# vrenkens/tfkaldi

Hardware: AMD Instinct MI355X
Metric: acoustic frames/sec (train step) (higher is better)
Workload: dtype f32 emulated (3xbf16 planes, 6 products, f32 accumulate)

## Files before the change

### tfkaldi_amd/csrc/engine.hip

```cpp
#include "../../include/tfkaldi_hip.h"
#include "ctc.h"
#include "gemm_bf16.h"
#include "gemm_f32.h"
#include "kernels.h"

#include <hip/hip_runtime.h>
#include <chrono>

#include <math.h>
#include <stdarg.h>
#include <stdlib.h>
#include <stdio.h>
#include <string.h>

#include <algorithm>
#include <string>
#include <vector>

using namespace tfk;

namespace {

thread_local std::string g_err;

// ... 61 lines not shown
  std::vector<hipEvent_t> ev_adam;
  bool opt_overlap = false;
  bool opt_pending = false;
  float* d_snap = nullptr;
  hipEvent_t ev_loss = nullptr;
  unsigned loss_seq = 0;
  bool loss_event = false;
  bool slot_lazy = true;
  hipEvent_t ev_grow = nullptr;
  std::vector<void*> host_garbage;

  float* state = nullptr;
  bool own_state = false;
  size_t P = 0, E = 0, state_floats = 0;
  size_t off_param = 0, off_grad = 0, off_scalars = 0, off_ema = 0, off_m = 0, off_v = 0, off_mov = 0, off_shadow = 0;
  size_t reduce_floats = 0;
  std::vector<LayerLayout> lay;

  int cap = 0;
  float* dX[2] = {nullptr, nullptr};
  int32_t* dY[2] = {nullptr, nullptr};
  std::vector<float*> z, a, v, rowscale, mean, rstd;
  float *logits = nullptr, *post = nullptr, *dA[2] = {nullptr, nullptr}, *row_loss = nullptr, *ws = nullptr;
  float* dRaw[2] = {nullptr, nullptr};
  int32_t* dSeg[2] = {nullptr, nullptr};
  float* hRaw[2] = {nullptr, nullptr};
  int32_t* hSeg[2] = {nullptr, nullptr};
  float* dCmvn[2] = {nullptr, nullptr};
  float* hCmvn[2] = {nullptr, nullptr};
  size_t cmvn_cap = 0;
  int seg_cap = 0;
  std::vector<float*> seg_mean, seg_rstd;
  float* ws_stats = nullptr;
  float* ws_bwd = nullptr;
  float* ws_splitk = nullptr;
  size_t ws_splitk_floats = 0;
  size_t ws_bwd_stride = 0;
  float* prior = nullptr;
  bool have_prior = false;

  float* hX[2] = {nullptr, nullptr};
  int32_t* hY[2] = {nullptr, nullptr};
  float* h_post = nullptr;
  size_t h_post_floats = 0;
  float* h_scalars = nullptr;
  float* h_scalars_dev = nullptr;
  bool apply_open = false, apply_direct = false;
  float cur_lr_t = 0.f;
  bool scalars_fresh = true;
  bool step_open = false;
  bool stash_live = false;
  float* scalar_stash = nullptr;
  bool colsum_done = false;
  bool fuse_hb_enabled = true;
  bool dual_gemm = true;
  bool stack_enabled = true;
  bool fuse_eval = true;
  int post_chunk = 2048;
  std::vector<hipEvent_t> post_ev;

  int32_t *ctc_seg = nullptr, *ctc_lab_off = nullptr, *ctc_lab = nullptr;
  float *ctc_lp = nullptr, *ctc_ab = nullptr, *ctc_bb = nullptr, *ctc_utt_loss = nullptr, *ctc_lse = nullptr;
  double *ctc_off = nullptr, *ctc_offb = nullptr, *ctc_logz = nullptr;
  size_t ctc_cap_bb = 0, ctc_cap_offb = 0, ctc_cap_logz = 0;
  int32_t* h_ctc[2] = {nullptr, nullptr};
  size_t h_ctc_cap[2] = {0, 0};
  hipEvent_t ctc_staged[2] = {nullptr, nullptr};
  int ctc_stage_slot = 0;
  size_t ctc_cap_offrows = 0;
  size_t ctc_cap_seg = 0, ctc_cap_off = 0, ctc_cap_loss = 0, ctc_cap_lab = 0, ctc_cap_lp = 0, ctc_cap_ab = 0,
         ctc_cap_rows = 0;
  int32_t* ctc_dec = nullptr;
  size_t ctc_cap_dec = 0;
  int32_t* h_dec = nullptr;
  size_t h_dec_cap = 0;
  unsigned long long* ctc_trie = nullptr;
  size_t ctc_cap_trie = 0;
  uint32_t* ctc_pre = nullptr;
  size_t ctc_cap_pre = 0;
  float* ctc_lm = nullptr;
  int ctc_lm_order = 0;
  unsigned char* ctc_bp = nullptr;
  size_t ctc_cap_bp = 0;
  unsigned char* ctc_sc = nullptr;
  size_t ctc_cap_sc = 0;
  int32_t* ctc_pair = nullptr;
  size_t ctc_cap_pair = 0;
  int32_t* h_pair = nullptr;
  size_t h_pair_cap = 0;
  hipEvent_t ctc_pair_staged = nullptr;

  bool bf16 = false;
  bool x3 = false;
  size_t tw_elems(size_t rows, int ld) const { return x3 ? x3::elems(rows, ld) : rows * ld; }
  size_t tw_row(size_t r, int ld) const { return x3 ? x3::at(r, 0, ld) : r * ld; }
  ShadowMap wb_map;
  int ldFb = 0, ldHb = 0, ldOb = 0;
  bf16_t* Xb[2] = {nullptr, nullptr};
  std::vector<bf16_t*> ab;
  bf16_t* logb = nullptr;
  bf16_t* dAb[2] = {nullptr, nullptr};
  bf16_t* Wb = nullptr;
  std::vector<size_t> wb_off;
  std::vector<int> wb_ld;
  bool wb_aligned = false;
  bool own_wb = false;
// ... 340 lines not shown
  auto frb = [&](bf16_t*& p) { dev_free(e, p, async); p = nullptr; };
  for (int s = 0; s < 2; ++s) { frb(e->Xb[s]); frb(e->dAb[s]); }
  for (auto& p : e->ab) frb(p);
  frb(e->logb);
  for (auto& p : e->z) fr(p);
  for (auto& p : e->a) fr(p);
  for (auto& p : e->v) fr(p);
  for (auto& p : e->rowscale) fr(p);
  fr(e->logits); fr(e->post); fr(e->row_loss); fr(e->ws); fr(e->ws_bwd); fr(e->ws_stats);
  e->cap = 0;
}

int alloc_zero(float** p, size_t floats) {
  HIPCHK(hipMalloc((void**)p, floats * sizeof(float)));
  HIPCHK(hipMemset(*p, 0, floats * sizeof(float)));
  HIPCHK(hipStreamSynchronize(nullptr));
  return 0;
}
int alloc_zero_b(bf16_t** p, size_t elems) {
  HIPCHK(hipMalloc((void**)p, elems * sizeof(bf16_t)));
  HIPCHK(hipMemset(*p, 0, elems * sizeof(bf16_t)));
  HIPCHK(hipStreamSynchronize(nullptr));
  return 0;
}
int grow_zero(tfk_engine* e, float** p, size_t floats) { return dev_alloc(e, (void**)p, floats * sizeof(float), true); }
int grow_zero_b(tfk_engine* e, bf16_t** p, size_t elems) { return dev_alloc(e, (void**)p, elems * sizeof(bf16_t), true); }

inline size_t seg_ints(int cap) { return (size_t)2 * cap + cap / 64 + 8; }

int reserve(tfk_engine* e, int T) {
  if (T <= e->cap) return 0;
  int cap = e->cap + e->cap / 2;
  if (cap < T) cap = T;
  cap = (int)up(cap, 64);
  for (int s = 0; s < 2; ++s)
    if (e->slot_used[s]) HIPCHK(hipEventSynchronize(e->copy_done[s]));
  free_activations(e, true);
  const int L = e->L;
  for (int s = 0; s < 2; ++s) {
    CHK(grow_zero(e, &e->dX[s], (size_t)cap * e->ldF));
    CHK(dev_alloc(e, (void**)&e->dY[s], (size_t)cap * sizeof(int32_t), false));
    CHK(grow_zero(e, &e->dA[s], (size_t)cap * e->ldH));
    HIPCHK(hipHostMalloc((void**)&e->hX[s], (size_t)cap * e->F * sizeof(float), hipHostMallocDefault));
    memset(e->hX[s], 0, (size_t)cap * e->F * sizeof(float));
    HIPCHK(hipHostMalloc((void**)&e->hY[s], (size_t)cap * sizeof(int32_t), hipHostMallocDefault));
    CHK(grow_zero(e, &e->dRaw[s], (size_t)cap * e->ldF));
    CHK(dev_alloc(e, (void**)&e->dSeg[s], seg_ints(cap) * sizeof(int32_t), false));
    HIPCHK(hipHostMalloc((void**)&e->hRaw[s], (size_t)cap * e->F * sizeof(float), hipHostMallocDefault));
    memset(e->hRaw[s], 0, (size_t)cap * e->F * sizeof(float));
    HIPCHK(hipHostMalloc((void**)&e->hSeg[s], seg_ints(cap) * sizeof(int32_t), hipHostMallocDefault));
    e->slot_used[s] = false;
  }
  e->z.assign(L, nullptr); e->a.assign(L, nullptr); e->v.assign(L, nullptr); e->rowscale.assign(L, nullptr);
  for (int l = 0; l < L; ++l) {
    CHK(grow_zero(e, &e->z[l], (size_t)cap * e->ldH));
    CHK(grow_zero(e, &e->a[l], (size_t)cap * e->ldH));
    if (e->cfg.l2_norm) {
      CHK(grow_zero(e, &e->v[l], (size_t)cap * e->ldH));
      CHK(grow_zero(e, &e->rowscale[l], (size_t)cap));
    }
  }
  if (e->bf16) {
    for (int s = 0; s < 2; ++s) {
      CHK(grow_zero_b(e, &e->Xb[s], e->tw_elems(cap, e->ldFb)));
      CHK(grow_zero_b(e, &e->dAb[s], e->tw_elems(cap, e->ldHb)));
    }
    e->ab.assign(L, nullptr);
    for (int l = 0; l < L; ++l) CHK(grow_zero_b(e, &e->ab[l], e->tw_elems(cap, e->ldHb)));
    CHK(grow_zero_b(e, &e->logb, e->tw_elems(cap, e->ldOb)));
  }
  CHK(grow_zero(e, &e->logits, (size_t)cap * e->ldO));
  CHK(grow_zero(e, &e->post, (size_t)cap * e->ldO));
  CHK(grow_zero(e, &e->row_loss, (size_t)cap));
  const int ldmax = e->ldH > e->ldO ? e->ldH : e->ldO;
  CHK(grow_zero(e, &e->ws, (size_t)3 * kMaxRowSplits * ldmax));
  CHK(grow_zero(e, &e->ws_stats, (size_t)2 * ((cap + 63) / 64) * e->ldH));
  e->ws_bwd_stride = (size_t)3 * kMaxRowSplits * ldmax;
  CHK(grow_zero(e, &e->ws_bwd, e->ws_bwd_stride * (L + 1)));
  HIPCHK(hipEventRecord(e->ev_grow, e->stream));
  HIPCHK(hipStreamWaitEvent(e->copy_stream, e->ev_grow, 0));
  e->cap = cap;
  return 0;
}

constexpr int kMaxStack = 32;
struct Stack {
  int k = 0;
  int r0[kMaxStack], rows[kMaxStack], span[kMaxStack];
  int T_pad = 0, T_valid = 0;
  const int* d_vend = nullptr;
};
int stack_align(const tfk_engine* e) { return (e->bf16 && !e->x3) ? 256 : 128; }

int wait_slot_free(tfk_engine* e, int s);
int stage_input(tfk_engine* e, const float* X, int64_t ldx, const int32_t* y, int T, int flags, const float** Xd,
                int* ldx_out, const int32_t** yd) {
  if (ldx < e->F) return fail(-1, "ldx %lld < input_dim %d", (long long)ldx, e->F);
  if (flags & TFK_DEVICE_PTRS) {
    if ((ldx % 4) == 0 && (e->F % 4) == 0 && (((uintptr_t)X) % 16) == 0) {
      *Xd = X;
      *ldx_out = (int)ldx;
    } else {
      const int s = e->slot;
      HIPCHK(hipMemcpy2DAsync(e->dX[s], (size_t)e->ldF * 4, X, (size_t)ldx * 4, (size_t)e->F * 4, T,
                              hipMemcpyDeviceToDevice, e->stream));
      *Xd = e->dX[s];
// ... 104 lines not shown
                  cmvn ? e->dCmvn[s] : nullptr, e->dX[s], e->ldF, st ? e->dSeg[s] + U + 1 : nullptr);
  }
  if (st) st->d_vend = e->dSeg[s] + 2 * U + 1;
  e->slot_used[s] = true;
  *Xd = e->dX[s];
  *ldx_out = e->ldF;
  *yd = e->dY[s];
  e->slot ^= 1;
  return 0;
}

int twin_input(tfk_engine* e, const float** Xd, int* ld, int T) {
  int s = (*Xd == e->dX[0]) ? 0 : (*Xd == e->dX[1]) ? 1 : -1;
  const float* src = *Xd;
  const int ld_src = *ld;
  if (s < 0) {
    s = e->slot;
    *Xd = e->dX[s];
    *ld = e->ldF;
  }
  to_bf16_rows(e->stream, src, ld_src, e->Xb[s], e->ldFb, T, e->F, e->x3);
  HIPCHK(hipGetLastError());
  return 0;
}

int finish_slot(tfk_engine* e, int flags, int slot_before) {
  if ((flags & TFK_DEVICE_PTRS) || e->slot == slot_before) return 0;
  if ((flags & TFK_LAST_MICROBATCH) && e->slot_lazy) {
    e->slot_step[slot_before] = e->steps_begun + 1;
    return 0;
  }
  e->slot_step[slot_before] = 0;
  HIPCHK(hipEventRecord(e->compute_done[slot_before], e->stream));
  return 0;
}
int wait_slot_free(tfk_engine* e, int s) {
  if (!e->slot_used[s]) return 0;
  if (e->slot_step[s] == 0) {
    HIPCHK(hipStreamWaitEvent(e->copy_stream, e->compute_done[s], 0));
  } else if (e->steps_seen < e->slot_step[s]) {
    HIPCHK(hipStreamSynchronize(e->stream));
  }
  return 0;
}

ActDesc act_desc(const tfk_engine* e, int layer, int train, uint32_t call) {
  ActDesc d;
  d.nonlin = e->cfg.nonlin; d.bn = e->cfg.batch_norm ? 1 : 0; d.l2 = e->cfg.l2_norm ? 1 : 0;
  d.keep = e->dropout ? e->cfg.keep_prob : 1.f;
  d.seed = e->cfg.seed; d.call = call; d.layer = (uint32_t)layer; d.train = train;
  return d;
}

int forward(tfk_engine* e, const float* Xd, int ldx, int T, int train, int nact, int nfw, uint32_t call,
            const Stack* st = nullptr) {
  const float* in = Xd;
  int ld_in = ldx;
  const int H = e->H, ldH = e->ldH;
  if (e->bf16 && e->shadow_dirty) {
    need_params(e, -1);
    CHK(join_optimizer(e));
    CHK(refresh_shadow(e));
  }
  auto twin_a = [&](int l) { Twin t; if (e->bf16) { t.p = e->ab[l]; t.ld = e->ldHb; t.x3 = e->x3; } return t; };
  for (int l = 0; l < nfw; ++l) {
    const LayerLayout& y = e->lay[l];
    need_params(e, l);
    CHK(wait_layer_update(e, l, l == 0));
    if (train && e->cfg.batch_norm && !e->cfg.l2_norm) {
      int cfg;
      const int chunk = gemm_chunk_rows(e, GEMM_NN, T, H, y.d_in, &cfg);
      if (st && stack_align(e) % chunk) return fail(-1, "internal: GEMM tile of %d rows does not divide the stack alignment", chunk);
      CHK(run_gemm(e, GEMM_NN, in, ld_in, e->p_param() + y.w_off, y.ld_out, e->z[l], ldH, T, H, y.d_in,
                   e->p_param() + y.b_off, EPI_BIAS | EPI_COLSTATS, nullptr, e->ws_stats, cfg, nullptr, st ? st->d_vend : nullptr));
      const int nchunk = (T + chunk - 1) / chunk;
      if (st) {
        for (int i = 0; i < st->k; ++i) {
          ProfScope ps(e, KF_ACT_FWD, 0, 8.0 * st->rows[i] * H);
          const ActDesc d = act_desc(e, l, train, call + (uint32_t)i);
          Twin tw = twin_a(l);
          if (e->bf16) tw.p += e->tw_row((size_t)st->r0[i], e->ldHb);
          bn_act_forward(e->stream, d, e->z[l] + (size_t)st->r0[i] * ldH, e->a[l] + (size_t)st->r0[i] * ldH,
                         e->ws_stats + (size_t)(st->r0[i] / chunk) * ldH, chunk, st->rows[i], H, ldH, e->bn_eps, e->bn_decay,
                         e->seg_mean[l] + (size_t)i * ldH, e->seg_rstd[l] + (size_t)i * ldH, e->ema_mean(l), e->ema_var(l),
                         e->p_param() + y.beta_off, tw, st->span[i], nchunk);
        }
      } else {
        ProfScope ps(e, KF_ACT_FWD, 0, 8.0 * T * H);
        const ActDesc d = act_desc(e, l, train, call);
        if (nchunk > kMergeOnceChunks && nchunk <= kMaxRowSplits) {
          bn_stats_from_chunks(e->stream, e->ws_stats, chunk, T, H, ldH, e->bn_eps, e->bn_decay, e->mean[l], e->rstd[l],
                               e->ema_mean(l), e->ema_var(l));
          act_forward(e->stream, d, e->z[l], e->a[l], nullptr, nullptr, e->mean[l], e->rstd[l],
                      e->p_param() + y.beta_off, T, H, ldH, twin_a(l));
        } else {
          bn_act_forward(e->stream, d, e->z[l], e->a[l], e->ws_stats, chunk, T, H, ldH, e->bn_eps,
                         e->bn_decay, e->mean[l], e->rstd[l], e->ema_mean(l), e->ema_var(l),
                         e->p_param() + y.beta_off, twin_a(l));
        }
      }
      in = e->a[l];
      ld_in = ldH;
      continue;
    }
    if (!train && !e->cfg.l2_norm && e->fuse_eval) {
      ActEpi ev = {nullptr, nullptr, e->cfg.batch_norm ? e->mov_mean(l) : nullptr,
                   e->cfg.batch_norm ? e->mov_var(l) : nullptr, e->cfg.nonlin};
      ev.beta = e->cfg.batch_norm ? e->p_param() + y.beta_off : nullptr;
      ev.eps = e->bn_eps;
      if (e->bf16) { ev.twin = e->ab[l]; ev.ld_twin = e->ldHb; }
      CHK(run_gemm(e, GEMM_NN, in, ld_in, e->p_param() + y.w_off, y.ld_out, e->a[l], ldH, T, H, y.d_in,
                   e->p_param() + y.b_off, EPI_BIAS | EPI_EVAL_ACT, nullptr, nullptr, -1, &ev));
      in = e->a[l];
      ld_in = ldH;
      continue;
    }
    CHK(run_gemm(e, GEMM_NN, in, ld_in, e->p_param() + y.w_off, y.ld_out, e->z[l], ldH, T, H, y.d_in,
                 e->p_param() + y.b_off, EPI_BIAS));
    if (e->cfg.batch_norm) {
      ProfScope ps(e, KF_BN_STATS, 0, 8.0 * T * H);
      if (train)
        bn_stats_train(e->stream, e->z[l], T, H, ldH, e->bn_eps, e->bn_decay, e->mean[l], e->rstd[l], e->ema_mean(l),
                       e->ema_var(l), e->ws);
      else
        bn_stats_eval(e->stream, e->mov_mean(l), e->mov_var(l), H, e->bn_eps, e->mean[l], e->rstd[l]);
    }
    {
      ProfScope ps(e, KF_ACT_FWD, 0, 8.0 * T * H);
      const ActDesc d = act_desc(e, l, train, call);
      act_forward(e->stream, d, e->z[l], e->a[l], e->cfg.l2_norm ? e->v[l] : nullptr,
                  e->cfg.l2_norm ? e->rowscale[l] : nullptr, e->mean[l], e->rstd[l],
                  e->cfg.batch_norm ? e->p_param() + y.beta_off : nullptr, T, H, ldH, twin_a(l));
    }
    in = e->a[l];
    ld_in = ldH;
  }
  const LayerLayout& o = e->lay[e->L];
  need_params(e, e->L);
  CHK(wait_layer_update(e, e->L, nfw == 0));
  CHK(run_gemm(e, GEMM_NN, e->a[nact - 1], ldH, e->p_param() + o.w_off, o.ld_out, e->logits, e->ldO, T, e->O, H,
               e->p_param() + o.b_off, EPI_BIAS));
  HIPCHK(hipGetLastError());
  return 0;
}

int backward(tfk_engine* e, const float* Xd, int ldx, int T, int nact, uint32_t call, bool fire, const Stack* st = nullptr) {
  const int L = e->L, H = e->H, ldH = e->ldH;
  const LayerLayout& o = e->lay[L];
  float* G = e->p_grad();
  const int acc = e->grads_fresh ? 0 : 1;
  const int epi_w = acc ? EPI_ACCUM : 0;
  if (!acc)
    for (int l = nact; l < L; ++l) {
      const LayerLayout& q = e->lay[l];
      HIPCHK(hipMemsetAsync(G + q.w_off, 0, q.w_sz * sizeof(float), e->stream));
      HIPCHK(hipMemsetAsync(G + q.b_off, 0, q.b_sz * sizeof(float), e->stream));
      if (q.beta_sz) HIPCHK(hipMemsetAsync(G + q.beta_off, 0, q.beta_sz * sizeof(float), e->stream));
    }
  FinalBatch fin;
  fin.n = 0;
  fin.accumulate = acc;
  const int rs = row_splits(T);
  auto ws_of = [&](int l) { return e->ws_bwd + (size_t)l * e->ws_bwd_stride; };
  {
    if (!e->colsum_done) {
      ProfScope ps(e, KF_COLSUM, 0, 4.0 * T * e->O);
      colsum_partial(e->stream, e->logits, T, e->ldO, ws_of(L));
    }
    e->colsum_done = false;
    fin.it[fin.n++] = {ws_of(L), G + o.b_off, 0, rs, e->O, e->ldO};
  }
  int pp = 0;
  int cfg_h, cfg_o;
  const int rows_h = gemm_chunk_rows(e, GEMM_NT, T, H, H, &cfg_h), rows_o = gemm_chunk_rows(e, GEMM_NT, T, H, e->O, &cfg_o);
  const bool drop = e->cfg.keep_prob < 1.f;
  const bool fuse_hb = e->cfg.batch_norm && !e->cfg.l2_norm && (!drop || e->cfg.nonlin == TFK_NONLIN_RELU) &&
                       e->fuse_hb_enabled && (T + rows_h - 1) / rows_h <= kMaxRowSplits &&
                       (T + rows_o - 1) / rows_o <= kMaxRowSplits;
  const std::vector<float*>& mean = st ? e->seg_mean : e->mean;
  const std::vector<float*>& rstd = st ? e->seg_rstd : e->rstd;
  auto act_of = [&](int l) {
    ActEpi act = {e->a[l], e->z[l], mean[l], rstd[l], e->cfg.nonlin};
    act.scale = drop ? 1.f / e->cfg.keep_prob : 1.f;
    act.beta = e->cfg.batch_norm ? e->p_param() + e->lay[l].beta_off : nullptr;
    return act;
  };
  auto dact_gemm = [&](const float* dz, int ld_dz, const float* W, int ldw, float* out, int K, int target, int cfg) {
    if (!fuse_hb) return run_gemm(e, GEMM_NT, dz, ld_dz, W, ldw, out, ldH, T, H, K, nullptr, 0);
    const ActEpi act = act_of(target);
    return run_gemm(e, GEMM_NT, dz, ld_dz, W, ldw, out, ldH, T, H, K, nullptr, EPI_DACT, nullptr, ws_of(target), cfg, &act);
  };
  int bm_in = rows_o;
  {
    const ActEpi act = act_of(nact - 1);
    const int rc = run_gemm_dual(e, e->logits, e->ldO, e->p_param() + o.w_off, o.ld_out, e->dA[pp], ldH, T, H, e->O,
                                 fuse_hb ? &act : nullptr, fuse_hb ? ws_of(nact - 1) : nullptr, e->a[nact - 1], ldH,
                                 G + o.w_off, o.ld_out, H, e->O, epi_w, &bm_in);
    if (rc < 0) return rc;
    if (rc > 0) {
      CHK(run_gemm(e, GEMM_TN, e->a[nact - 1], ldH, e->logits, e->ldO, G + o.w_off, o.ld_out, H, e->O, T, nullptr, epi_w));
      CHK(dact_gemm(e->logits, e->ldO, e->p_param() + o.w_off, o.ld_out, e->dA[pp], e->O, nact - 1, cfg_o));
    }
  }
  if (fire && e->cb) {
    e->cb(e->cb_user, 0);
    for (int l = L - 1; l >= nact; --l) e->cb(e->cb_user, L - l);
  }
  for (int l = nact - 1; l >= 0; --l) {
    const LayerLayout& y = e->lay[l];
    float* da = e->dA[pp];
    const int chunks_in = (T + bm_in - 1) / bm_in;
    auto fin_layer = [&](int n_beta, int n_bias) {
      if (e->cfg.batch_norm) fin.it[fin.n++] = {ws_of(l), G + y.beta_off, 0, n_beta, H, ldH};
      fin.it[fin.n++] = {ws_of(l), G + y.b_off, 2, n_bias, H, ldH};
      if (fin.n + 2 > kMaxFinalItems) {
        grad_final(e->stream, fin);
        fin.n = 0;
      }
    };
    Twin tw;
    if (e->bf16) { tw.p = e->dAb[pp]; tw.ld = e->ldHb; tw.x3 = e->x3; }
    if (st) {
      if (!fuse_hb || stack_align(e) % bm_in || chunks_in > kMaxRowSplits)
        return fail(-1, "internal: EPI_DACT chunks of %d rows do not fit a stacked pass of %d rows", bm_in, T);
      int slot = 0;
      for (int i = 0; i < st->k; ++i) {
        ProfScope ps(e, KF_HIDDEN_BWD, 0, 28.0 * st->rows[i] * H);
        const ActDesc d = act_desc(e, l, 1, call + (uint32_t)i);
        Twin tws = tw;
        if (e->bf16) tws.p += e->tw_row((size_t)st->r0[i], e->ldHb);
        const size_t r = (size_t)st->r0[i] * ldH;
        hidden_backward(e->stream, d, 1, da + r, e->a[l] + r, e->z[l] + r, mean[l] + (size_t)i * ldH, rstd[l] + (size_t)i * ldH,
                        st->rows[i], H, ldH, ws_of(l) + (size_t)(st->r0[i] / bm_in) * ldH, (st->rows[i] + bm_in - 1) / bm_in, tws,
                        st->span[i], ws_of(l) + ((size_t)2 * kMaxRowSplits + slot) * ldH);
        slot += row_splits(st->span[i]);
// ... 1876 lines not shown
  return 0;
}

int tfk_profile_begin(tfk_engine* e) {
  if (!e) return fail(-1, "engine is NULL");
  e->prof.clear();
  e->ev_next = 0;
  e->profiling = true;
  return 0;
}
int tfk_profile_end(tfk_engine* e, tfk_kernel_stat* stats, int capacity, int* count) {
  if (!e || !count) return fail(-1, "NULL argument");
  HIPCHK(hipSetDevice(e->cfg.device));
  CHK(sync_streams(e));
  e->profiling = false;
  tfk_kernel_stat acc[KF_COUNT];
  memset(acc, 0, sizeof(acc));
  for (int f = 0; f < KF_COUNT; ++f) snprintf(acc[f].name, sizeof(acc[f].name), "%s", kFamilyName[f]);
  for (const ProfRec& r : e->prof) {
    float ms = 0.f;
    HIPCHK(hipEventElapsedTime(&ms, r.a, r.b));
    acc[r.family].launches += 1;
    acc[r.family].total_ms += ms;
    acc[r.family].flops += r.flops;
    acc[r.family].bytes += r.bytes;
  }
  int n = 0;
  for (int f = 0; f < KF_COUNT; ++f)
    if (acc[f].launches > 0) {
      if (stats && n < capacity) stats[n] = acc[f];
      ++n;
    }
  *count = n;
  e->prof.clear();
  e->ev_next = 0;
  return 0;
}

int tfk_debug_fetch(tfk_engine* e, int what, int layer, float* host, size_t count) {
  if (!e || !host) return fail(-1, "NULL argument");
  HIPCHK(hipSetDevice(e->cfg.device));
  CHK(sync_streams(e));
  const int T = e->last_T;
  if (T <= 0) return fail(-1, "no previous call to fetch from");
  if (what == TFK_DBG_LOGITS) {
    if (count != (size_t)T * e->O) return fail(-1, "count %zu != %d x %d", count, T, e->O);
    HIPCHK(hipMemcpy2D(host, (size_t)e->O * 4, e->logits, (size_t)e->ldO * 4, (size_t)e->O * 4, T, hipMemcpyDeviceToHost));
    return 0;
  }
  if (layer < 0 || layer >= e->L) return fail(-1, "layer %d out of range", layer);
  if (count != (size_t)T * e->H) return fail(-1, "count %zu != %d x %d", count, T, e->H);
  if (what == TFK_DBG_HIDDEN) {
    if (layer >= e->last_nfw) return fail(-1, "layer %d was not evaluated by the last call", layer);
    HIPCHK(hipMemcpy2D(host, (size_t)e->H * 4, e->a[layer], (size_t)e->ldH * 4, (size_t)e->H * 4, T, hipMemcpyDeviceToHost));
    return 0;
  }
  if (what == TFK_DBG_PREACT || what == TFK_DBG_BN_MEAN || what == TFK_DBG_BN_RSTD) {
    if (what == TFK_DBG_PREACT) {
      HIPCHK(hipMemcpy2D(host, (size_t)e->H * 4, e->z[layer], (size_t)e->ldH * 4, (size_t)e->H * 4, T, hipMemcpyDeviceToHost));
    } else {
      memset(host, 0, count * sizeof(float));
      HIPCHK(hipMemcpy(host, what == TFK_DBG_BN_MEAN ? e->mean[layer] : e->rstd[layer], (size_t)e->H * 4, hipMemcpyDeviceToHost));
    }
    return 0;
  }
  if (what == TFK_DBG_DROPOUT_MASK) {
    const ActDesc d = act_desc(e, layer, 1, e->last_call);
    if (d.keep >= 1.f) {
      for (size_t i = 0; i < count; ++i) host[i] = 1.f;
      return 0;
    }
    dropout_mask(e->stream, d, e->dA[0], T, e->H, e->ldH);
    HIPCHK(hipStreamSynchronize(e->stream));
    HIPCHK(hipMemcpy2D(host, (size_t)e->H * 4, e->dA[0], (size_t)e->ldH * 4, (size_t)e->H * 4, T, hipMemcpyDeviceToHost));
    return 0;
  }
  return fail(-1, "unknown debug tensor %d", what);
}

int tfk_gemm_f32(void* stream, int layout, const float* A, int lda, const float* B, int ldb, float* C, int ldc, int M,
                 int N, int K, const float* bias, int epi, int tile_config) {
  if (layout < 0 || layout > 2) return fail(-1, "bad layout %d", layout);
  GemmArgs g;
  g.A = A; g.B = B; g.C = C; g.bias = bias; g.stats = nullptr;
  g.act_a = g.act_z = g.act_mean = g.act_rstd = nullptr; g.act_nonlin = 0; g.stats_stride = 0;
  g.M = M; g.N = N; g.K = K; g.lda = lda; g.ldb = ldb; g.ldc = ldc; g.epi = epi;
  const int rc = gemm_f32((GemmLayout)layout, g, tile_config, (hipStream_t)stream);
  if (rc != 0) return fail(rc, "gemm_f32 failed: %s", hipGetErrorString((hipError_t)rc));
  return 0;
}

int tfk_gemm_bf16(void* stream, int layout, const uint16_t* A, int lda, const uint16_t* B, int ldb, float* C, int ldc,
                  int M, int N, int K, const float* bias, int epi) {
  if (layout < 0 || layout > 2) return fail(-1, "bad layout %d", layout);
  GemmArgsB g = {};
  g.A = A; g.B = B; g.C = C; g.bias = bias;
  g.M = M; g.N = N; g.K = K; g.lda = lda; g.ldb = ldb; g.ldc = ldc; g.epi = epi;
  const int rc = gemm_bf16((GemmLayout)layout, g, (hipStream_t)stream);
  if (rc != 0) return fail(rc, "gemm_bf16 failed: %s", hipGetErrorString((hipError_t)rc));
  return 0;
}

int tfk_split3(void* stream, const float* src, int lds, uint16_t* dst, int ldd, int rows, int cols) {
  if (!src || !dst) return fail(-1, "NULL argument");
  if ((ldd & 31) || ldd < cols) return fail(-1, "tfk_split3: ldd %d (a multiple of 32, >= cols)", ldd);
  to_bf16_rows((hipStream_t)stream, src, lds, dst, ldd, rows, cols, 1);
// ... 76 lines not shown
```

### tfkaldi_amd/csrc/gemm_bf16.hip

```cpp
#include "gemm_bf16.h"
#include "x3_layout.h"

#include <math.h>
#include <stdlib.h>
#include <string.h>

#include <type_traits>

namespace tfk {
namespace {

typedef __bf16 bf16x8 __attribute__((ext_vector_type(8)));
typedef __bf16 bf16x4 __attribute__((ext_vector_type(4)));
typedef float f32x16 __attribute__((ext_vector_type(16)));
typedef uint32_t u32x4 __attribute__((ext_vector_type(4)));
typedef int i32x4 __attribute__((ext_vector_type(4)));

constexpr int BK = 64;
constexpr int kOOB = (int)0x80000000;
constexpr int NUM_XCD = 8;

__device__ __forceinline__ void tile_of_seq(int tiles_m, int tiles_n, int group_rows, int seq, int& tm, int& tn) {
  const int per_group = group_rows * tiles_n;
  const int grp = seq / per_group;
// ... 36 lines not shown
      const float mu = bn ? p.act_mean[colc] : 0.f;
      const float rs = bn ? rsqrtf(p.act_rstd[colc] + p.bn_eps) : 1.f;
      const float be = bn ? p.act_beta[colc] : 0.f;
#pragma unroll
      for (int a = 0; a < FM; ++a)
#pragma unroll
        for (int r = 0; r < 16; ++r) {
          float u = acc[a][b][r];
          if (bn) u = (u - mu) * rs + be;
          switch (p.act_nonlin) {
            case 0: u = fmaxf(u, 0.f); break;
            case 1: u = 1.f / (1.f + expf(-u)); break;
            case 2: u = tanhf(u); break;
            default: break;
          }
          acc[a][b][r] = u;
        }
    }
    if constexpr ((EPI & EPI_COLSTATS) != 0) {
      const int vlim = p.row_vend ? min(p.M, p.row_vend[m0 >> 6]) : p.M;
      const int n_tile = max(1, min(BM, vlim - m0));
      float cmean = 0.f;
#pragma unroll
      for (int pass = 0; pass < 2; ++pass) {
        float s = 0.f;
#pragma unroll
        for (int a = 0; a < FM; ++a)
#pragma unroll
          for (int r = 0; r < 16; ++r) {
            const float v = acc[a][b][r];
            if (row_of(a, r) < vlim) s += pass == 0 ? v : (v - cmean) * (v - cmean);
          }
        s += __shfl_xor(s, 32);
        if (h == 0) red[wm * BN + cidx] = s;
        __syncthreads();
        float t = 0.f;
#pragma unroll
        for (int w = 0; w < WAVES_M; ++w) t += red[w * BN + cidx];
        if (pass == 0) {
          cmean = t / (float)n_tile;
        } else if (wm == 0 && h == 0 && col_ok) {
          p.stats[((size_t)0 * tiles_m + tm) * p.ldc + col] = cmean;
          p.stats[((size_t)1 * tiles_m + tm) * p.ldc + col] = t;
        }
        __syncthreads();
      }
    }
    if constexpr ((EPI & EPI_DACT) != 0) {
      const float mu = p.act_mean[colc], rsd = p.act_rstd[colc];
      const float dscale = p.act_scale > 0.f ? p.act_scale : 1.f;
      const bool from_a = p.act_nonlin == 0 && p.act_beta != nullptr;
      const float be = from_a ? p.act_beta[colc] : 0.f;
      const float keep = p.act_keep > 0.f ? p.act_keep : 1.f;
      float s1 = 0.f, s2 = 0.f;
#pragma unroll
      for (int a = 0; a < FM; ++a) {
        float av[16], zv[16];
#pragma unroll
        for (int r = 0; r < 16; ++r) {
          const int row = min(row_of(a, r), p.M - 1);
          av[r] = p.act_a[(size_t)row * p.ldc + colc];
        }
        if (!from_a) {
#pragma unroll
          for (int r = 0; r < 16; ++r) {
            const int row = min(row_of(a, r), p.M - 1);
            zv[r] = p.act_z[(size_t)row * p.ldc + colc];
          }
        }
#pragma unroll
        for (int r = 0; r < 16; ++r) {
          float d1;
          switch (p.act_nonlin) {
            case 0: d1 = av[r] > 0.f ? dscale : 0.f; break;
            case 1: d1 = av[r] * (1.f - av[r]); break;
            case 2: d1 = 1.f - av[r] * av[r]; break;
            default: d1 = 1.f;
          }
          const float du = acc[a][b][r] * d1;
          acc[a][b][r] = du;
          if (row_of(a, r) < p.M) {
            s1 += du;
            s2 += du * (from_a ? av[r] * keep - be : (zv[r] - mu) * rsd);
          }
        }
      }
      s1 += __shfl_xor(s1, 32);
      s2 += __shfl_xor(s2, 32);
      if (h == 0) {
        red[(0 * WAVES_M + wm) * BN + cidx] = s1;
        red[(1 * WAVES_M + wm) * BN + cidx] = s2;
      }
      __syncthreads();
      if (wm == 0 && h == 0 && col_ok) {
        float t1 = 0.f, t2 = 0.f;
#pragma unroll
        for (int w = 0; w < WAVES_M; ++w) {
          t1 += red[(0 * WAVES_M + w) * BN + cidx];
          t2 += red[(1 * WAVES_M + w) * BN + cidx];
        }
        p.stats[((size_t)0 * p.stats_stride + tm) * p.ldc + col] = t1;
        p.stats[((size_t)1 * p.stats_stride + tm) * p.ldc + col] = t2;
      }
      __syncthreads();
    }
    if constexpr (CBUF) {
      static_assert((EPI & EPI_EVAL_ACT) == 0, "no bf16 twin on this path");
      const __amdgpu_buffer_rsrc_t crs =
          __builtin_amdgcn_make_buffer_rsrc((void*)p.C, 0, (int)(((unsigned)(p.M - 1) * p.ldc + p.N) * 4u), 0x00020000);
#pragma unroll
      for (int a = 0; a < FM; ++a) {
        const unsigned base = col_ok ? ((unsigned)(m0 + (wm * FM + a) * 32 + 4 * h) * p.ldc + col) * 4u : (unsigned)kOOB;
        float old[16];
        if constexpr ((EPI & EPI_ACCUM) != 0) {
// ... 1162 lines not shown
```

### tfkaldi_amd/csrc/kernels.hip

```cpp
#include "kernels.h"

#include <math.h>
#include <stdlib.h>

namespace tfk {
namespace {

constexpr int NONLIN_RELU = 0, NONLIN_SIGMOID = 1, NONLIN_TANH = 2, NONLIN_LINEAR = 3;

__device__ __forceinline__ float wave_sum(float v) {
#pragma unroll
  for (int o = 32; o > 0; o >>= 1) v += __shfl_xor(v, o);
  return v;
}
__device__ __forceinline__ float wave_max(float v) {
#pragma unroll
  for (int o = 32; o > 0; o >>= 1) v = fmaxf(v, __shfl_xor(v, o));
  return v;
}
__device__ __forceinline__ float block_sum(float v, float* sm) {
  v = wave_sum(v);
  const int w = threadIdx.x >> 6, nw = blockDim.x >> 6;
  if ((threadIdx.x & 63) == 0) sm[w] = v;
  __syncthreads();
// ... 233 lines not shown
#pragma unroll
  for (int k = 0; k < FIN_KL; ++k) acc += sm[k][threadIdx.x];
  const float mu = acc / (float)T;
  __syncthreads();
  float m2 = 0.f;
#pragma unroll
  for (int j = 0; j < FIN_PER; ++j) {
    const float d = mk[j] - mu;
    m2 += qk[j] + nk[j] * d * d;
  }
  sm[ky][threadIdx.x] = m2;
  __syncthreads();
  if (ky != 0 || c >= ld) return;
  if (!live) {
    mean[c] = 0.f; rstd[c] = 0.f;
    return;
  }
  acc = 0.f;
#pragma unroll
  for (int k = 0; k < FIN_KL; ++k) acc += sm[k][threadIdx.x];
  const float var = acc / (float)T;
  mean[c] = mu;
  rstd[c] = rsqrtf(var + eps);
  e_mean[c] = decay * e_mean[c] + (1.f - decay) * mu;
  e_var[c] = decay * e_var[c] + (1.f - decay) * var;
}

__global__ void bn_stats_eval_kernel(const float* __restrict__ mov_mean, const float* __restrict__ mov_var, int H,
                                     float eps, float* __restrict__ mean, float* __restrict__ rstd) {
  const int c = blockIdx.x * blockDim.x + threadIdx.x;
  if (c >= H) return;
  mean[c] = mov_mean[c];
  rstd[c] = rsqrtf(mov_var[c] + eps);
}

template <bool L2>
__global__ void __launch_bounds__(256)
act_forward_kernel(ActDesc d, const float* __restrict__ z, float* __restrict__ a, float* __restrict__ vbuf,
                   float* __restrict__ rowscale, const float* __restrict__ mean, const float* __restrict__ rstd,
                   const float* __restrict__ beta, int T, int H, int ld, Twin tw) {
  __shared__ float sm[4];
  const int nc4 = ld >> 2;
  const bool drop = d.train && d.keep < 1.f;
  const float inv_keep = drop ? 1.f / d.keep : 1.f;
  for (int row = blockIdx.x; row < T; row += gridDim.x) {
    const float* zr = z + (size_t)row * ld;
    float* ar = a + (size_t)row * ld;
    float ss = 0.f;
    for (int c4 = threadIdx.x; c4 < nc4; c4 += blockDim.x) {
      const int col = c4 << 2;
      float4 u = ld4(zr + col);
      if (d.bn) {
        const float4 mu = ld4(mean + col), rs = ld4(rstd + col), be = ld4(beta + col);
        u.x = (u.x - mu.x) * rs.x + be.x; u.y = (u.y - mu.y) * rs.y + be.y;
        u.z = (u.z - mu.z) * rs.z + be.z; u.w = (u.w - mu.w) * rs.w + be.w;
      }
      float4 v;
#pragma unroll
      for (int k = 0; k < 4; ++k) el(v, k) = (col + k < H) ? nonlin_fwd(el(u, k), d.nonlin) : 0.f;
      if (L2) {
        ss += v.x * v.x + v.y * v.y + v.z * v.z + v.w * v.w;
        st4(vbuf + (size_t)row * ld + col, v);
      } else {
        if (drop) {
          const Keep4 m = keep_mask(d, row, c4);
#pragma unroll
          for (int k = 0; k < 4; ++k) el(v, k) = m.k[k] ? el(v, k) * inv_keep : 0.f;
        }
        st4(ar + col, v);
        st4_twin(tw, row, col, v);
      }
    }
    if (L2) {
      const float s = block_sum(ss, sm) / (float)H;
      if (threadIdx.x == 0) rowscale[row] = s;
      const float scale = s > 1.f ? 1.f / s : 1.f;
      for (int c4 = threadIdx.x; c4 < nc4; c4 += blockDim.x) {
        const int col = c4 << 2;
        float4 v = ld4(vbuf + (size_t)row * ld + col);
        v.x *= scale; v.y *= scale; v.z *= scale; v.w *= scale;
        if (drop) {
          const Keep4 m = keep_mask(d, row, c4);
#pragma unroll
          for (int k = 0; k < 4; ++k) el(v, k) = m.k[k] ? el(v, k) * inv_keep : 0.f;
        }
        st4(ar + col, v);
        st4_twin(tw, row, col, v);
      }
    }
  }
}

__global__ void __launch_bounds__(CT_X * CT_Y)
bn_act_forward_kernel(ActDesc d, const float* __restrict__ z, float* __restrict__ a, const float* __restrict__ st,
                      int nchunk, int chunk_rows, int T, int H, int ld, int rows_per, float eps, float decay,
                      float* __restrict__ mean, float* __restrict__ rstd, float* __restrict__ e_mean,
                      float* __restrict__ e_var, const float* __restrict__ beta, Twin tw, int T_apply, int slab, int nt) {
  __shared__ float4 sm[CT_Y][CT_X];
  __shared__ float4 smm[CT_X];
  const ColTile t = col_tile(T_apply, ld, rows_per);
  const float4 zero4 = make_float4(0.f, 0.f, 0.f, 0.f);
  constexpr int KREG = 2;
  const bool in_regs = nchunk <= KREG * CT_Y;
  float4 mreg[KREG], qreg[KREG];
  float nreg[KREG];
#pragma unroll
  for (int j = 0; j < KREG; ++j) {
    const int k = threadIdx.y + j * CT_Y;
// ... 39 lines not shown
  }
  if (!in_regs && t.valid)
    for (int k = threadIdx.y + KREG * CT_Y; k < nchunk; k += CT_Y) {
      const float n = (float)max(min(T, (k + 1) * chunk_rows) - k * chunk_rows, 0);
      const float4 m = ld4(st + ((size_t)0 * slab + k) * ld + t.col);
      const float4 q = ld4(st + ((size_t)1 * slab + k) * ld + t.col);
      m2.x += q.x + n * (m.x - mu.x) * (m.x - mu.x); m2.y += q.y + n * (m.y - mu.y) * (m.y - mu.y);
      m2.z += q.z + n * (m.z - mu.z) * (m.z - mu.z); m2.w += q.w + n * (m.w - mu.w) * (m.w - mu.w);
    }
  m2 = reduce_rows(m2, sm);
  if (threadIdx.y == 0) {
    const float inv = 1.f / (float)T;
    float4 var = make_float4(m2.x * inv, m2.y * inv, m2.z * inv, m2.w * inv);
    float4 rs4;
#pragma unroll
    for (int k = 0; k < 4; ++k) el(rs4, k) = (t.col + k < H) ? rsqrtf(el(var, k) + eps) : 0.f;
    smm[threadIdx.x] = rs4;
    if (blockIdx.y == 0 && t.valid) {
      float4 mu_w = mu;
#pragma unroll
      for (int k = 0; k < 4; ++k)
        if (t.col + k >= H) el(mu_w, k) = 0.f;
      st4(mean + t.col, mu_w);
      st4(rstd + t.col, rs4);
      float4 em = ld4(e_mean + t.col), ev = ld4(e_var + t.col);
#pragma unroll
      for (int k = 0; k < 4; ++k)
        if (t.col + k < H) {
          el(em, k) = decay * el(em, k) + (1.f - decay) * el(mu, k);
          el(ev, k) = decay * el(ev, k) + (1.f - decay) * el(var, k);
        }
      st4(e_mean + t.col, em);
      st4(e_var + t.col, ev);
    }
  }
  __syncthreads();
  if (!t.valid) return;
  const float4 rsd = smm[threadIdx.x];
  const bool drop = d.train && d.keep < 1.f;
  const float inv_keep = drop ? 1.f / d.keep : 1.f;
  for (int rb = rb0; rb < t.r1; rb += CT_Y * RB) {
    float4 zn[RB];
    const int rbn = rb + CT_Y * RB;
#pragma unroll
    for (int j = 0; j < RB; ++j) {
      const int r = rbn + j * CT_Y;
      zn[j] = rbn < t.r1 ? ld4s(z + (size_t)(r < t.r1 ? r : rbn) * ld + t.col, nt) : zero4;
    }
#pragma unroll
    for (int j = 0; j < RB; ++j) {
      const int r = rb + j * CT_Y;
      if (r >= t.r1) continue;
      float4 v;
      v.x = (zv[j].x - mu.x) * rsd.x + be.x; v.y = (zv[j].y - mu.y) * rsd.y + be.y;
      v.z = (zv[j].z - mu.z) * rsd.z + be.z; v.w = (zv[j].w - mu.w) * rsd.w + be.w;
#pragma unroll
      for (int k = 0; k < 4; ++k) el(v, k) = (t.col + k < H) ? nonlin_fwd(el(v, k), d.nonlin) : 0.f;
      if (drop) {
        const Keep4 m = keep_mask(d, r, t.c4);
#pragma unroll
        for (int k = 0; k < 4; ++k) el(v, k) = m.k[k] ? el(v, k) * inv_keep : 0.f;
      }
      if (nt & 1) st4_nt(a + (size_t)r * ld + t.col, v);
      else st4(a + (size_t)r * ld + t.col, v);
      if (nt & 2) st4_twin_nt(tw, r, t.col, v);
      else st4_twin(tw, r, t.col, v);
    }
#pragma unroll
    for (int j = 0; j < RB; ++j) zv[j] = zn[j];
  }
}

__global__ void __launch_bounds__(256)
act_backward_rows_kernel(ActDesc d, float* __restrict__ da, const float* __restrict__ vbuf,
                         const float* __restrict__ rowscale, int T, int H, int ld) {
  __shared__ float sm[4];
  const int nc4 = ld >> 2;
  const bool drop = d.keep < 1.f;
  const float inv_keep = drop ? 1.f / d.keep : 1.f;
  for (int row = blockIdx.x; row < T; row += gridDim.x) {
    float* gr = da + (size_t)row * ld;
    const float* vr = vbuf + (size_t)row * ld;
    const float s = rowscale[row];
    float dot = 0.f;
    if (s > 1.f) {
      for (int c4 = threadIdx.x; c4 < nc4; c4 += blockDim.x) {
        const int col = c4 << 2;
        float4 g = ld4(gr + col);
        const float4 v = ld4(vr + col);
        if (drop) {
          const Keep4 m = keep_mask(d, row, c4);
#pragma unroll
          for (int k = 0; k < 4; ++k) el(g, k) = m.k[k] ? el(g, k) * inv_keep : 0.f;
        }
        dot += g.x * v.x + g.y * v.y + g.z * v.z + g.w * v.w;
      }
      dot = block_sum(dot, sm);
    }
    const float k1 = s > 1.f ? 1.f / s : 1.f;
    const float k2 = s > 1.f ? 2.f * dot / ((float)H * s * s) : 0.f;
    for (int c4 = threadIdx.x; c4 < nc4; c4 += blockDim.x) {
      const int col = c4 << 2;
      float4 g = ld4(gr + col);
      const float4 v = ld4(vr + col);
      if (drop) {
        const Keep4 m = keep_mask(d, row, c4);
#pragma unroll
        for (int k = 0; k < 4; ++k) el(g, k) = m.k[k] ? el(g, k) * inv_keep : 0.f;
      }
      float4 o;
#pragma unroll
      for (int k = 0; k < 4; ++k) {
        const float dv = el(g, k) * k1 - el(v, k) * k2;
        el(o, k) = (col + k < H) ? dv * nonlin_bwd(el(v, k), d.nonlin) : 0.f;
      }
      st4(gr + col, o);
    }
// ... 807 lines not shown
```

### tfkaldi_amd/csrc/x3_layout.h

```cpp
#pragma once
#include <stddef.h>
#include <stdint.h>

#if defined(__HIPCC__)
#define X3_HD __host__ __device__ __forceinline__
#else
#define X3_HD inline
#endif

namespace tfk {
namespace x3 {

constexpr int kSlotK = 32;

X3_HD size_t elems(size_t rows, int ld) { return ((rows + 1) >> 1) * (size_t)(ld >> 5) * 192; }
X3_HD size_t at(size_t row, int col, int ld) {
  return ((row >> 1) * (size_t)(ld >> 5) + (size_t)(col >> 5)) * 192 + (row & 1) * 32 + (col & 31);
}

X3_HD int kc_swz(int r) { return (r >> 2) & 3; }
X3_HD void kc_decode(int n, int& r, int& q, int& c) {
  const int P = n / 24, rem = n - P * 24;
  q = rem >> 3;
  r = 2 * P + ((rem >> 2) & 1);
// ... 25 lines not shown
  const int kb = lane >> 5, half = (lane >> 4) & 1, j = (lane >> 2) & 3, qq = lane & 3;
  const int t = (j >> 1) & 1;
  const int base = (4 * kb + (j >> 1)) * (EXT / 32 * 384) + (j & 1) * 64 + (2 * half + (qq >> 1)) * 16 + ((qq & 1) << 3) +
                   128 * 3 * frag0;
  const int xt_odd = (frag0 + x_odd) & 1;
  return base + (xt_odd ? -128 * t : 128 * t) + (x_odd ? 128 : 0);
}
template <int EXT>
X3_HD int ks_imm(int X, int ks, int hi) {
  return 128 * (X & ~1) + (ks * 8 + hi * 2) * (EXT / 32 * 384);
}

constexpr int kXcds = 8;
constexpr int kCus = 256;
X3_HD int dual_tiles_per_block(int n_long, int nk_long, int n_short, int nk_short) {
  int per = (nk_long + (nk_short - 1) / 2) / nk_short;
  if (per < 1) per = 1;
  while (per > 1 && n_long + (n_short + per - 1) / per < kCus) --per;
  return per;
}
X3_HD void dual_block_tiles(int n_short, int per, int g, int& seq0, int& count) {
  const int xcd = g % kXcds, j = g / kXcds;
  const int q = n_short / kXcds, r = n_short % kXcds;
  const int start = xcd < r ? xcd * (q + 1) : r * (q + 1) + (xcd - r) * q;
  const int cnt = q + (xcd < r ? 1 : 0);
  const int left = cnt - j * per;
  seq0 = start + j * per;
  count = left <= 0 ? 0 : left < per ? left : per;
}
X3_HD int dual_short_blocks(int n_short, int per) {
  const int q = n_short / kXcds, r = n_short % kXcds;
  if (q == 0) return r;
  const int j_q = (q + per - 1) / per, j_q1 = (q + 1 + per - 1) / per;
  return (r > 0 && j_q1 > j_q) ? kXcds * j_q + r : kXcds * j_q;
}

#if defined(__HIPCC__)
__device__ __forceinline__ void split3(float x, uint16_t& p1, uint16_t& p2, uint16_t& p3) {
  const uint32_t ux = __builtin_bit_cast(uint32_t, x);
  uint32_t b1 = (uint32_t)__builtin_bit_cast(uint16_t, (__bf16)x) << 16;
  const bool edge = (b1 & 0x7fffffffu) == 0x7f800000u && (ux & 0x7fffffffu) < 0x7f800000u;
  if (edge) b1 = ux & 0xffff0000u;
  const float r1 = x - __builtin_bit_cast(float, b1);
  uint32_t b2 = (uint32_t)__builtin_bit_cast(uint16_t, (__bf16)r1) << 16;
  if (edge) b2 = __builtin_bit_cast(uint32_t, r1) & 0xffff0000u;
  const float r2 = r1 - __builtin_bit_cast(float, b2);
  p1 = (uint16_t)(b1 >> 16);
  p2 = (uint16_t)(b2 >> 16);
  p3 = (uint16_t)(__builtin_bit_cast(uint32_t, r2) >> 16);
}
#endif

}
}
```

Baseline: 961,200.

## Skip storing fp32 hidden activations in BN+ReLU training; recompute from z in backward

```diff
diff --git a/tfkaldi_amd/csrc/engine.hip b/tfkaldi_amd/csrc/engine.hip
--- a/tfkaldi_amd/csrc/engine.hip
+++ b/tfkaldi_amd/csrc/engine.hip
@@ -137,6 +137,8 @@
   bool stash_live = false;
   float* scalar_stash = nullptr;
   bool colsum_done = false;
+  std::vector<char> a_current;
+  unsigned long long a_pass_step = 0;
   bool fuse_hb_enabled = true;
   bool dual_gemm = true;
   bool stack_enabled = true;
@@ -583,6 +585,7 @@
     e->slot_used[s] = false;
   }
   e->z.assign(L, nullptr); e->a.assign(L, nullptr); e->v.assign(L, nullptr); e->rowscale.assign(L, nullptr);
+  e->a_current.assign(L, 1);
   for (int l = 0; l < L; ++l) {
     CHK(grow_zero(e, &e->z[l], (size_t)cap * e->ldH));
     CHK(grow_zero(e, &e->a[l], (size_t)cap * e->ldH));
@@ -793,6 +796,24 @@
   return d;
 }
 
+struct FuseHb {
+  bool on;
+  int rows_h, cfg_h, rows_o, cfg_o;
+};
+FuseHb fuse_hb_of(tfk_engine* e, int T) {
+  FuseHb f;
+  f.rows_h = gemm_chunk_rows(e, GEMM_NT, T, e->H, e->H, &f.cfg_h);
+  f.rows_o = gemm_chunk_rows(e, GEMM_NT, T, e->H, e->O, &f.cfg_o);
+  const bool drop = e->cfg.keep_prob < 1.f;
+  f.on = e->cfg.batch_norm && !e->cfg.l2_norm && (!drop || e->cfg.nonlin == TFK_NONLIN_RELU) && e->fuse_hb_enabled &&
+         (T + f.rows_h - 1) / f.rows_h <= kMaxRowSplits && (T + f.rows_o - 1) / f.rows_o <= kMaxRowSplits;
+  return f;
+}
+bool act_copy_forced() {
+  static const bool on = [] { const char* v = getenv("TFK_ACT_COPY"); return v && atoi(v) != 0; }();
+  return on;
+}
+
 int forward(tfk_engine* e, const float* Xd, int ldx, int T, int train, int nact, int nfw, uint32_t call,
             const Stack* st = nullptr) {
   const float* in = Xd;
@@ -804,8 +825,12 @@
     CHK(refresh_shadow(e));
   }
   auto twin_a = [&](int l) { Twin t; if (e->bf16) { t.p = e->ab[l]; t.ld = e->ldHb; t.x3 = e->x3; } return t; };
+  const bool skip_copy = train && !st && e->bf16 && e->cfg.batch_norm && !e->cfg.l2_norm && e->cfg.nonlin == TFK_NONLIN_RELU &&
+                         e->cfg.keep_prob >= 1.f && !act_copy_forced() && fuse_hb_of(e, T).on;
+  e->a_pass_step = e->steps_begun;
   for (int l = 0; l < nfw; ++l) {
     const LayerLayout& y = e->lay[l];
+    e->a_current[l] = 1;
     need_params(e, l);
     CHK(wait_layer_update(e, l, l == 0));
     if (train && e->cfg.batch_norm && !e->cfg.l2_norm) {
@@ -835,9 +860,10 @@
           act_forward(e->stream, d, e->z[l], e->a[l], nullptr, nullptr, e->mean[l], e->rstd[l],
                       e->p_param() + y.beta_off, T, H, ldH, twin_a(l));
         } else {
-          bn_act_forward(e->stream, d, e->z[l], e->a[l], e->ws_stats, chunk, T, H, ldH, e->bn_eps,
+          bn_act_forward(e->stream, d, e->z[l], skip_copy ? nullptr : e->a[l], e->ws_stats, chunk, T, H, ldH, e->bn_eps,
                          e->bn_decay, e->mean[l], e->rstd[l], e->ema_mean(l), e->ema_var(l),
                          e->p_param() + y.beta_off, twin_a(l));
+          if (skip_copy) e->a_current[l] = 0;
         }
       }
       in = e->a[l];
@@ -912,16 +938,17 @@
     fin.it[fin.n++] = {ws_of(L), G + o.b_off, 0, rs, e->O, e->ldO};
   }
   int pp = 0;
-  int cfg_h, cfg_o;
-  const int rows_h = gemm_chunk_rows(e, GEMM_NT, T, H, H, &cfg_h), rows_o = gemm_chunk_rows(e, GEMM_NT, T, H, e->O, &cfg_o);
+  const FuseHb fh = fuse_hb_of(e, T);
+  const int cfg_h = fh.cfg_h, cfg_o = fh.cfg_o, rows_h = fh.rows_h, rows_o = fh.rows_o;
   const bool drop = e->cfg.keep_prob < 1.f;
-  const bool fuse_hb = e->cfg.batch_norm && !e->cfg.l2_norm && (!drop || e->cfg.nonlin == TFK_NONLIN_RELU) &&
-                       e->fuse_hb_enabled && (T + rows_h - 1) / rows_h <= kMaxRowSplits &&
-                       (T + rows_o - 1) / rows_o <= kMaxRowSplits;
+  const bool fuse_hb = fh.on;
+  for (int l = 0; l < nact; ++l)
+    if (!e->a_current[l] && (!fuse_hb || st || !e->bf16))
+      return fail(-1, "internal: the backward pass needs the fp32 output of layer %d, which the forward pass did not store", l);
   const std::vector<float*>& mean = st ? e->seg_mean : e->mean;
   const std::vector<float*>& rstd = st ? e->seg_rstd : e->rstd;
   auto act_of = [&](int l) {
-    ActEpi act = {e->a[l], e->z[l], mean[l], rstd[l], e->cfg.nonlin};
+    ActEpi act = {e->a_current[l] ? e->a[l] : nullptr, e->z[l], mean[l], rstd[l], e->cfg.nonlin};
     act.scale = drop ? 1.f / e->cfg.keep_prob : 1.f;
     act.beta = e->cfg.batch_norm ? e->p_param() + e->lay[l].beta_off : nullptr;
     return act;
@@ -2904,6 +2931,18 @@
   if (count != (size_t)T * e->H) return fail(-1, "count %zu != %d x %d", count, T, e->H);
   if (what == TFK_DBG_HIDDEN) {
     if (layer >= e->last_nfw) return fail(-1, "layer %d was not evaluated by the last call", layer);
+    if (!e->a_current[layer]) {
+      if (e->a_pass_step != e->steps_begun || e->shadow_dirty)
+        return fail(-1, "the last training call's output of layer %d was not kept and the parameters have changed since "
+                        "(fetch it before the optimiser step, or set TFK_ACT_COPY=1)", layer);
+      ActDesc d = act_desc(e, layer, 1, e->last_call);
+      d.keep = 1.f;
+      act_forward(e->stream, d, e->z[layer], e->a[layer], nullptr, nullptr, e->mean[layer], e->rstd[layer],
+                  e->p_param() + e->lay[layer].beta_off, T, e->H, e->ldH, Twin());
+      HIPCHK(hipGetLastError());
+      HIPCHK(hipStreamSynchronize(e->stream));
+      e->a_current[layer] = 1;
+    }
     HIPCHK(hipMemcpy2D(host, (size_t)e->H * 4, e->a[layer], (size_t)e->ldH * 4, (size_t)e->H * 4, T, hipMemcpyDeviceToHost));
     return 0;
   }
diff --git a/tfkaldi_amd/csrc/gemm_bf16.hip b/tfkaldi_amd/csrc/gemm_bf16.hip
--- a/tfkaldi_amd/csrc/gemm_bf16.hip
+++ b/tfkaldi_amd/csrc/gemm_bf16.hip
@@ -112,6 +112,8 @@
       const bool from_a = p.act_nonlin == 0 && p.act_beta != nullptr;
       const float be = from_a ? p.act_beta[colc] : 0.f;
       const float keep = p.act_keep > 0.f ? p.act_keep : 1.f;
+      const bool from_z = from_a && p.act_a == nullptr;
+      const float* __restrict__ src = from_z ? p.act_z : p.act_a;
       float s1 = 0.f, s2 = 0.f;
 #pragma unroll
       for (int a = 0; a < FM; ++a) {
@@ -119,7 +121,11 @@
 #pragma unroll
         for (int r = 0; r < 16; ++r) {
           const int row = min(row_of(a, r), p.M - 1);
-          av[r] = p.act_a[(size_t)row * p.ldc + colc];
+          av[r] = src[(size_t)row * p.ldc + colc];
+        }
+        if (from_z) {
+#pragma unroll
+          for (int r = 0; r < 16; ++r) av[r] = fmaxf(bn_affine(av[r], mu, rsd, be), 0.f);
         }
         if (!from_a) {
 #pragma unroll
diff --git a/tfkaldi_amd/csrc/kernels.hip b/tfkaldi_amd/csrc/kernels.hip
--- a/tfkaldi_amd/csrc/kernels.hip
+++ b/tfkaldi_amd/csrc/kernels.hip
@@ -309,8 +309,8 @@
       float4 u = ld4(zr + col);
       if (d.bn) {
         const float4 mu = ld4(mean + col), rs = ld4(rstd + col), be = ld4(beta + col);
-        u.x = (u.x - mu.x) * rs.x + be.x; u.y = (u.y - mu.y) * rs.y + be.y;
-        u.z = (u.z - mu.z) * rs.z + be.z; u.w = (u.w - mu.w) * rs.w + be.w;
+        u.x = bn_affine(u.x, mu.x, rs.x, be.x); u.y = bn_affine(u.y, mu.y, rs.y, be.y);
+        u.z = bn_affine(u.z, mu.z, rs.z, be.z); u.w = bn_affine(u.w, mu.w, rs.w, be.w);
       }
       float4 v;
 #pragma unroll
@@ -456,8 +456,8 @@
       const int r = rb + j * CT_Y;
       if (r >= t.r1) continue;
       float4 v;
-      v.x = (zv[j].x - mu.x) * rsd.x + be.x; v.y = (zv[j].y - mu.y) * rsd.y + be.y;
-      v.z = (zv[j].z - mu.z) * rsd.z + be.z; v.w = (zv[j].w - mu.w) * rsd.w + be.w;
+      v.x = bn_affine(zv[j].x, mu.x, rsd.x, be.x); v.y = bn_affine(zv[j].y, mu.y, rsd.y, be.y);
+      v.z = bn_affine(zv[j].z, mu.z, rsd.z, be.z); v.w = bn_affine(zv[j].w, mu.w, rsd.w, be.w);
 #pragma unroll
       for (int k = 0; k < 4; ++k) el(v, k) = (t.col + k < H) ? nonlin_fwd(el(v, k), d.nonlin) : 0.f;
       if (drop) {
@@ -465,8 +465,10 @@
 #pragma unroll
         for (int k = 0; k < 4; ++k) el(v, k) = m.k[k] ? el(v, k) * inv_keep : 0.f;
       }
-      if (nt & 1) st4_nt(a + (size_t)r * ld + t.col, v);
-      else st4(a + (size_t)r * ld + t.col, v);
+      if (a) {
+        if (nt & 1) st4_nt(a + (size_t)r * ld + t.col, v);
+        else st4(a + (size_t)r * ld + t.col, v);
+      }
       if (nt & 2) st4_twin_nt(tw, r, t.col, v);
       else st4_twin(tw, r, t.col, v);
     }
diff --git a/tfkaldi_amd/csrc/x3_layout.h b/tfkaldi_amd/csrc/x3_layout.h
--- a/tfkaldi_amd/csrc/x3_layout.h
+++ b/tfkaldi_amd/csrc/x3_layout.h
@@ -101,4 +101,10 @@
 #endif
 
 }
+
+#if defined(__HIPCC__)
+__device__ __forceinline__ float bn_affine(float z, float mean, float rstd, float beta) {
+  return __fmaf_rn(__fsub_rn(z, mean), rstd, beta);
 }
+#endif
+}
```

Result: no change. 967,200 (median of 6 runs) (+0.6%).
